# mauro3/KissMCMC.jl

Measured on AMD Instinct MI355X. Metric: walker-steps/sec, higher is better.
Workload: dtype f64

## Files before the change

include/kissmcmc_hip.h:

```cpp
#ifndef KISSMCMC_HIP_H
#define KISSMCMC_HIP_H

#include <stdint.h>

#ifdef __cplusplus
extern "C" {
#endif

#define KMC_VERSION 100

typedef enum kmc_status {
    KMC_OK = 0,
    KMC_ERR_A_SCALE = 1,
    KMC_ERR_ODD_WALKERS = 2,
    KMC_ERR_TOO_FEW_WALKERS = 3,
    KMC_ERR_BAD_ARG = 4,
    KMC_ERR_NONFINITE_LOGP = 5,
    KMC_ERR_HIP = 6,
    KMC_ERR_OOM = 7,
    KMC_ERR_NO_DEVICE = 8,
    KMC_ERR_UNSUPPORTED = 9
} kmc_status;

typedef enum kmc_density {
// ... 413 lines not shown
kmc_status  kmc_chain_psis_tail_reff(kmc_user_density* density, const double* params, const double* chain_host, int64_t nsamples, int64_t nwalkers,
                                     int64_t ndim, int64_t first_sample, const uint8_t* walker_mask, int64_t thin, const double* r_eff_j,
                                     int32_t split, int64_t max_lag, int64_t obs_first, int64_t obs_count, int64_t workspace_bytes, int device,
                                     double* tail, double* m_j, double* xc_j, int32_t* n_tail_j, int64_t* tail_len, double* r_eff_used,
                                     int64_t* tail_len_j, int64_t* n_reff_nan, int64_t* n_out);

kmc_status  kmc_debug_accept_terms(uint64_t seed, uint64_t step, uint64_t walker0, int64_t n, int64_t nhalf, double a_scale,
                                   int64_t ndim, int device, int64_t* partner_host, double* z_host, double* t1_host, double* lu_host);
kmc_status  kmc_debug_chain_by_walker(const void* src_host, int is_float, int64_t K, int64_t nl, int64_t ld, int64_t nd, int64_t w0,
                                      int64_t nw, int64_t dst_stride, double* dst_host, int64_t dst_len, int device);
kmc_status  kmc_debug_rows_compact(const double* src_host, int64_t rows, int64_t ld, int64_t nd, double* dst_host, int64_t dst_len,
                                   int device);
int         kmc_debug_phase_spec(int density, int L, int K, int iter);
int         kmc_debug_shared_draws(int density, int L, int K, int iter);
int         kmc_debug_replay_variant(int density, int64_t nwalkers, int64_t ndim, int64_t nburnin, int64_t g0, int64_t n, int moments, int chain);

#ifdef __cplusplus
}
#endif
#endif
```

kissmcmc.jl_amd/_lib.py:

```python
from __future__ import annotations

import ctypes as C
import os

_HERE = os.path.dirname(os.path.abspath(__file__))
LIB_PATH = os.environ.get("KMC_LIB_PATH") or os.path.join(_HERE, "libkissmcmc_hip.so")

OK, ERR_A_SCALE, ERR_ODD_WALKERS, ERR_TOO_FEW_WALKERS, ERR_BAD_ARG, ERR_NONFINITE_LOGP, \
    ERR_HIP, ERR_OOM, ERR_NO_DEVICE, ERR_UNSUPPORTED = range(10)
GAUSSIAN_ISO, EXPONENTIAL, ROSENBROCK, LOGNORMAL, MVNORMAL2 = range(5)
USER_DENSITY = 100
HOST_DENSITY = 101
DATA_DENSITY = 102
HOST_LOGPDF_FN = C.CFUNCTYPE(C.c_int, C.POINTER(C.c_double), C.c_int64, C.c_int64, C.POINTER(C.c_double), C.c_void_p)
HOST_PROPOSE_FN = C.CFUNCTYPE(C.c_int, C.POINTER(C.c_double), C.c_int64, C.c_int64, C.POINTER(C.c_double), C.c_void_p)
HOST_ACCEPTED_FN = C.CFUNCTYPE(C.c_int, C.POINTER(C.c_uint8), C.c_int64, C.c_int64, C.c_int64, C.c_int32, C.c_void_p)
F64 = 0
F32 = 1
STORE_CHAIN, STORE_LOGP, MOMENTS, NO_GRAPH, P2P, ISLANDS, P2P_FINEGRAINED, P2P_PUSH = 1, 2, 4, 8, 16, 64, 128, 512
STREAM_CHAIN = 2048
CHAIN_BY_WALKER = 4096
STORE_BLOBS = 8192
MOVE_STRETCH, MOVE_DE, MOVE_SNOOKER, MOVE_MIX = 0, 1, 3, 4
MIX_MAX = 4
# ... 5 lines not shown
RCCL_ID_BYTES = 128

SYMBOLS = [
    "kmc_version", "kmc_device_count", "kmc_last_error", "kmc_status_string", "kmc_validate",
    "kmc_g_pdf", "kmc_cdf_g_inv", "kmc_emcee_run", "kmc_sampler_create", "kmc_sampler_destroy",
    "kmc_sampler_set_stream", "kmc_sampler_bind_positions", "kmc_sampler_p2p_export", "kmc_sampler_p2p_connect", "kmc_sampler_p2p_connect_local", "kmc_sampler_p2p_link_probe", "kmc_sampler_set_positions", "kmc_sampler_init_ball", "kmc_sampler_set_state", "kmc_sampler_run", "kmc_sampler_half_step",
    "kmc_sampler_sync", "kmc_sampler_last_run_ms", "kmc_sampler_generation", "kmc_sampler_nsamples",
    "kmc_sampler_launch_count", "kmc_sampler_describe", "kmc_sampler_device_ptr", "kmc_sampler_get_positions",
    "kmc_sampler_get_logp", "kmc_sampler_get_naccept", "kmc_sampler_get_accept_ratio",
    "kmc_sampler_get_moments", "kmc_sampler_get_chain", "kmc_sampler_get_chain_by_walker", "kmc_logpdf_eval", "kmc_logpdf_eval_host",
    "kmc_user_density_create", "kmc_user_density_create_body", "kmc_user_density_destroy", "kmc_metropolis_validate", "kmc_metropolis_run", "kmc_cholesky_lower", "kmc_int_acorr", "kmc_sampler_int_acorr",
    "kmc_sizeof_config", "kmc_sizeof_metropolis_config", "kmc_sizeof_outputs", "kmc_sizeof_metropolis_outputs", "kmc_deal_seed", "kmc_deal_perm", "kmc_sampler_deal_pack", "kmc_sampler_deal_unpack",
    "kmc_sampler_get_walker_ids", "kmc_sampler_set_walker_ids", "kmc_sampler_set_chain_host", "kmc_rccl_unique_id", "kmc_sampler_rccl_init",
    "kmc_sampler_rccl_capture", "kmc_sampler_rccl_set_capture", "kmc_rccl_version", "kmc_device_free_bytes",
    "kmc_sampler_launch_mode", "kmc_updated_budget", "kmc_set_updated_budget_mb", "kmc_debug_accept_terms",
    "kmc_debug_chain_by_walker", "kmc_debug_rows_compact", "kmc_debug_phase_spec", "kmc_debug_shared_draws", "kmc_debug_replay_variant",
    "kmc_user_density_create_body_blob", "kmc_user_density_nblob", "kmc_logpdf_blob_eval_host", "kmc_sampler_get_blobs",
    "kmc_device_cache_release", "kmc_user_density_is_separable", "kmc_host_prefault", "kmc_data_density_create",
    "kmc_sampler_get_rung_state", "kmc_sampler_set_rung_state", "kmc_sampler_get_swaps",
    "kmc_sampler_get_rung_loglike", "kmc_sampler_set_rung_loglike_sum", "kmc_sampler_get_ladder", "kmc_sampler_set_ladder",
    "kmc_sampler_order_stats", "kmc_sampler_chain_argmax", "kmc_chain_order_stats", "kmc_chain_argmax",
    "kmc_sampler_histograms", "kmc_chain_histograms", "kmc_hist_pair_plan",
    "kmc_sampler_lag_sums", "kmc_chain_lag_sums", "kmc_convergence_stats", "kmc_sampler_convergence", "kmc_chain_convergence",
    "kmc_convergence_plan",
    "kmc_rank_plan", "kmc_rank_normal_scores", "kmc_sampler_rank_scores", "kmc_chain_rank_scores", "kmc_sampler_rank_convergence",
    "kmc_chain_rank_convergence",
    "kmc_sampler_hdi", "kmc_chain_hdi", "kmc_hdi_span",
    "kmc_sampler_covariance", "kmc_chain_covariance", "kmc_cov_plan", "kmc_cov_correlation",
    "kmc_sampler_pointwise_stats", "kmc_chain_pointwise_stats", "kmc_sampler_pointwise_loglike", "kmc_chain_pointwise_loglike",
    "kmc_pointwise_plan", "kmc_waic_stats",
    "kmc_sampler_psis_loo", "kmc_chain_psis_loo", "kmc_sampler_psis_tail", "kmc_chain_psis_tail", "kmc_psis_plan", "kmc_loo_stats",
# ... 285 lines not shown
    L.kmc_sampler_launch_mode.restype = C.c_int
    L.kmc_sampler_launch_mode.argtypes = [vp, C.POINTER(C.c_int)]
    L.kmc_updated_budget.restype = None
    L.kmc_updated_budget.argtypes = [ip, ip]
    L.kmc_set_updated_budget_mb.restype = None
    L.kmc_set_updated_budget_mb.argtypes = [C.c_double]
    L.kmc_debug_accept_terms.argtypes = [C.c_uint64, C.c_uint64, C.c_uint64, C.c_int64, C.c_int64, C.c_double, C.c_int64, C.c_int, ip, dp, dp, dp]
    L.kmc_debug_chain_by_walker.argtypes = [vp, C.c_int, C.c_int64, C.c_int64, C.c_int64, C.c_int64, C.c_int64, C.c_int64, C.c_int64, dp, C.c_int64, C.c_int]
    L.kmc_debug_rows_compact.argtypes = [dp, C.c_int64, C.c_int64, C.c_int64, dp, C.c_int64, C.c_int]
    L.kmc_debug_phase_spec.restype = C.c_int
    L.kmc_debug_phase_spec.argtypes = [C.c_int, C.c_int, C.c_int, C.c_int]
    L.kmc_debug_shared_draws.restype = C.c_int
    L.kmc_debug_shared_draws.argtypes = [C.c_int, C.c_int, C.c_int, C.c_int]
    L.kmc_debug_replay_variant.restype = C.c_int
    L.kmc_debug_replay_variant.argtypes = [C.c_int, C.c_int64, C.c_int64, C.c_int64, C.c_int64, C.c_int64, C.c_int, C.c_int]
    for fn, T in ((L.kmc_sizeof_config, Config), (L.kmc_sizeof_metropolis_config, MetropolisConfig),
                  (L.kmc_sizeof_outputs, Outputs), (L.kmc_sizeof_metropolis_outputs, MetropolisOutputs)):
        if fn() != C.sizeof(T):
            raise ImportError(f"{LIB_PATH}: struct layout mismatch ({fn.__name__}() = {fn()}, the ctypes mirror {T.__name__} is {C.sizeof(T)} bytes): "
                              "rebuild the library or update kissmcmc_jl_amd/_lib.py from include/kissmcmc_hip.h")
    _lib = L
    return L


def check(status: int) -> None:
    if status != OK:
        L = lib()
        msg = L.kmc_last_error().decode() or L.kmc_status_string(status).decode()
        raise KmcError(status, msg)
```

kissmcmc.jl_amd/build.py:

```python
from __future__ import annotations

import os
import shutil
import subprocess

_HERE = os.path.dirname(os.path.abspath(__file__))
CSRC = os.path.join(_HERE, "csrc")
LIB = os.path.join(_HERE, "libkissmcmc_hip.so")
SOURCES = ["kmc_sampler.hip", "kmc_validate.hip", "kmc_describe.hip", "kmc_plan.hip", "kmc_launch.hip", "kmc_updated.hip", "kmc_state.hip", "kmc_copy.hip", "kmc_rtc.hip", "kmc_p2p.hip", "kmc_metropolis_api.hip", "kmc_acorr.hip", "kmc_summary.hip", "kmc_hist.hip", "kmc_convergence.hip", "kmc_rank.hip", "kmc_hdi.hip", "kmc_cov.hip", "kmc_pointwise.hip", "kmc_rccl.hip", "kmc_diag.hip", "kmc_inst_host.hip", "kmc_inst_host_temper.hip", "kmc_inst_host_temper_snooker.hip", "kmc_data.hip"] + \
          [f"kmc_inst_{d}{part}.hip" for part in ("", "_var", "_p2p", "_lds", "_spec", "_share", "_de", "_snooker", "_temper", "_temper_snooker") for d in ("lognormal", "exponential", "gaussian_iso", "rosenbrock", "mvnormal2")
           if (part, d) != ("_share", "mvnormal2")]
HEADERS = ["kmc_psis_fit.hpp", "kmc_host.hpp", "kmc_sampler.hpp", "kmc_device.hpp", "kmc_kernels.hpp", "kmc_islands.hpp", "kmc_generation.hpp", "kmc_copy_kernels.hpp", "kmc_summary_kernels.hpp", "kmc_hist_kernels.hpp", "kmc_convergence_kernels.hpp", "kmc_convergence_host.hpp", "kmc_rank_kernels.hpp", "kmc_rank_host.hpp", "kmc_hdi_kernels.hpp", "kmc_cov_kernels.hpp", "kmc_chain_view.hpp", "kmc_chain_kernels.hpp", "kmc_metropolis.hpp", "kmc_tables.hpp", "kmc_shared_draws.hpp", "kmc_recognise.hpp", "kmc_data.hpp", "kmc_pointwise.hpp", os.path.join("..", "..", "include", "kissmcmc_hip.h")]
PRELOAD = ["-mllvm", "-amdgpu-kernarg-preload-count=14"]
FLAGS = ["--offload-arch=gfx950", "-O3", "-std=c++17", "-fPIC", "-ffp-contract=off",
         "-fvisibility=hidden", "-Wall", "-Wno-unused-function"]


def _hipcc() -> str:
    for c in (shutil.which("hipcc"), "/opt/rocm/bin/hipcc"):
        if c and os.path.exists(c):
            return c
    raise RuntimeError("hipcc not found: the HIP library cannot be built")




def stale(lib: str = LIB) -> bool:
# ... 38 lines not shown
```

kissmcmc.jl_amd/csrc/kmc_describe.hip:

```cpp
#include <cstdio>
#include <sstream>

#include "kmc_sampler.hpp"

using namespace kmc;
using namespace kmc_host;

namespace {
std::string launch_mode_text(const kmc_sampler* s, const char* what)
{
    std::string t = ((s->cfg.flags & KMC_NO_GRAPH) || s->launch_mode == 2) ? std::string(", eager launches (") + what + " among the preloaded kernel parameters)"
                    : s->launch_mode == 3 ? ", hipGraph replay of " + std::to_string(s->uchunk) + " generations with per-replay parameter updates (" + what + " preloaded)"
                                          : std::string(", hipGraph replay of 64 generations");
    if (s->calib_graph_ms > 0.f) {
        char b[128];
        std::snprintf(b, sizeof(b), " (measured per 64 generations: table graph %.3f ms, %s %.3f ms)", s->calib_graph_ms, s->launch_mode == 2 ? "eager launches" : "updated graph", s->calib_eager_ms);
        t += b;
    }
    return t;
}

void write_islands(std::ostringstream& o, const kmc_sampler* s)
{
    o << "island mode: " << s->nislands << " islands of " << s->island_size << " walkers in LDS, " << s->island_gens
// ... 51 lines not shown
}
void write_route(std::ostringstream& o, const kmc_sampler* s)
{
    if (s->islands) write_islands(o, s);
    else if (s->resident) write_resident(o, s);
    else if (s->fused) write_generation(o, s);
    else if (s->data_eval) write_data_density(o, s);
    else if (s->host_eval) write_host_density(o, s);
    else if (s->plan.vec) write_two_launch_vec(o, s);
    else write_two_launch_generic(o, s);
}

void write_feed_stats(std::ostringstream& o, const kmc_sampler* s)
{
    if (s->feed_replays <= 0 || !debug_opt("feed-stats")) return;
    char b[200];
    std::snprintf(b, sizeof(b), "; feeding thread per replay of %lld generations: wait for a free executable %.1f us, parameter updates %.1f us, hipGraphLaunch %.1f us (%lld replays)",
                  (long long)s->uchunk, s->feed_wait_ns / 1e3 / s->feed_replays, s->feed_update_ns / 1e3 / s->feed_replays, s->feed_launch_ns / 1e3 / s->feed_replays, (long long)s->feed_replays);
    o << b;
}

std::string move_kernel(const kmc_sampler* s, const char* stem)
{
    const std::string k = std::string("half_step_") + stem;
    return s->host_eval ? k + "_generic (propose / accept passes)" : s->plan.vec ? k + "_vec" : k + "_generic";
}
void write_move(std::ostringstream& o, const kmc_sampler* s)
{
    char b[160];
    if (s->cfg.move == KMC_MOVE_DE) {
        std::snprintf(b, sizeof(b), "; differential-evolution move (KMC_MOVE_DE): gamma0 %.6g, sigma %.3g, kernel ", de_gamma0_of(s->cfg), s->cfg.de_sigma);
        o << b << move_kernel(s, "de");
    }
    if (s->cfg.move == KMC_MOVE_SNOOKER) {
// ... 85 lines not shown
}
}

KMC_EXPORT kmc_status kmc_sampler_describe(const kmc_sampler* s, char* buf, int64_t buflen)
{
    if (!s || !buf || buflen <= 0) return fail(KMC_ERR_BAD_ARG, "bad argument");
    std::ostringstream o;
    write_route(o, s);
    write_feed_stats(o, s);
    write_move(o, s);
    write_tempering(o, s);
    write_storage(o, s);
    write_density(o, s);
    write_shard(o, s);
    write_geometry(o, s);
    const std::string t = o.str();
    std::snprintf(buf, (size_t)buflen, "%s", t.c_str());
    return KMC_OK;
}
```

kissmcmc.jl_amd/csrc/kmc_launch.hip:

```cpp
#include <algorithm>
#include <cmath>
#include <cstdio>
#include <cstdlib>

#define KMC_DEFINE_LAUNCH_KERNELS
#include "kmc_sampler.hpp"

using namespace kmc;
using namespace kmc_host;

namespace kmc_host {

template <int L, int K, int ITER, class T>
FlushFn flush_one()
{
    if constexpr (ITER <= L && ITER * K <= 16) return flush_moments_vec<L, K, ITER, T>;
    else return nullptr;
}

template <int L, int K>
FlushFn flush_iter(int iter, bool f32)
{
    switch (iter) {
    case 1: return f32 ? flush_one<L, K, 1, float>() : flush_one<L, K, 1, double>();
// ... 561 lines not shown
{
    if (s->fused) HIP_TRY(generation_settle(s));
    KMC_TRY(ensure_graph(s));
    if (!s->graph_exec) return eager_generations(s, kGraphChunk, left);
    KMC_TRY(sync_device_counter(s));
    KMC_TRY(chain_before(s, s->generation + kGraphChunk));
    HIP_TRY(hipGraphLaunch(s->graph_exec, s->stream));
    if (!s->fused) HIP_TRY(launch_sweep(s));
    s->generation += kGraphChunk;
    s->dev_gen += kGraphChunk;
    s->launches += (launches_per_generation(s) + (s->temper ? 1 : 0)) * kGraphChunk;
    *left -= kGraphChunk;
    return chain_after(s);
}

kmc_status updated_chunk(kmc_sampler* s, int64_t* left)
{
    if (s->fused) HIP_TRY(generation_settle(s));
    KMC_TRY(chain_before(s, s->generation + s->uchunk));
    bool launched = false;
    if (launch_updated_graph(s, &launched) != KMC_OK) {
        s->launch_mode = 1;
        if (debug_opt("feed-stats")) std::fprintf(stderr, "[kissmcmc_hip] the updated-graph replay failed (%s): table graph from here on\n", kmc_last_error());
        if (!launched) return KMC_OK;
        HIP_TRY(hipStreamSynchronize(s->stream));
    }
    if (!s->fused) HIP_TRY(launch_sweep(s));
    s->generation += s->uchunk;
    s->launches += launches_per_generation(s) * s->uchunk;
    *left -= s->uchunk;
    return chain_after(s);
}

inline int64_t calib_gens(const kmc_sampler* s) { return std::max<int64_t>(4 * kGraphChunk, 2 * s->uchunk); }
inline int64_t calib_min(const kmc_sampler* s) { return kGraphChunk + 2 * std::max<int64_t>(kGraphChunk, s->uchunk) + 2 * calib_gens(s) + kGraphChunk; }

kmc_status calibrate(kmc_sampler* s, bool with_updated, int64_t* left)
{
    hipEvent_t e0 = nullptr, e1 = nullptr, e2 = nullptr;
    HIP_TRY(hipEventCreate(&e0));
    HIP_TRY(hipEventCreate(&e1));
    HIP_TRY(hipEventCreate(&e2));
    const int64_t gens = calib_gens(s);
    kmc_status st = graph_chunk(s, left);
    if (st == KMC_OK) st = with_updated ? updated_chunk(s, left) : eager_generations(s, kGraphChunk, left);
    if (st == KMC_OK) st = with_updated ? updated_chunk(s, left) : eager_generations(s, kGraphChunk, left);
    if (st == KMC_OK && hipEventRecord(e0, s->stream) != hipSuccess) st = KMC_ERR_HIP;
    for (int64_t r = 0; r < gens / kGraphChunk && st == KMC_OK; ++r) st = graph_chunk(s, left);
    if (st == KMC_OK && hipEventRecord(e1, s->stream) != hipSuccess) st = KMC_ERR_HIP;
    if (with_updated) { for (int64_t r = 0; r < gens / s->uchunk && st == KMC_OK && s->launch_mode == 0; ++r) st = updated_chunk(s, left); }
    else if (st == KMC_OK) st = eager_generations(s, gens, left);
    if (st == KMC_OK && hipEventRecord(e2, s->stream) != hipSuccess) st = KMC_ERR_HIP;
    float tg = 0.f, tu = 0.f;
    if (st == KMC_OK && (hipEventSynchronize(e2) != hipSuccess || hipEventElapsedTime(&tg, e0, e1) != hipSuccess ||
                         hipEventElapsedTime(&tu, e1, e2) != hipSuccess)) st = KMC_ERR_HIP;
    (void)hipEventDestroy(e0); (void)hipEventDestroy(e1); (void)hipEventDestroy(e2);
    if (st != KMC_OK) return st == KMC_ERR_HIP ? fail(st, "launch-mode calibration failed") : st;
    if (s->launch_mode == 0) {
        s->launch_mode = tu < 0.98f * tg ? (with_updated ? 3 : 2) : 1;
        s->calib_graph_ms = tg * (float)kGraphChunk / (float)gens; s->calib_eager_ms = tu * (float)kGraphChunk / (float)gens;
    }
    return KMC_OK;
}

enum class LaunchEnv { none, graph, eager, updated, updated_budget };
LaunchEnv launch_env()
{
    static const char* const names[] = {"graph", "eager", "updated", "updated,budget"};
    const char* const e = std::getenv("KMC_LAUNCH");
    for (int i = 0; e && i < 4; ++i)
        if (std::strcmp(e, names[i]) == 0) return (LaunchEnv)(i + 1);
    return LaunchEnv::none;
}

kmc_status decide_launch_mode(kmc_sampler* s, LaunchEnv env, bool use_graph, int64_t* left)
{
    constexpr int64_t kWorthMeasuring = 4096;
    const bool long_job = s->cfg.ngenerations >= kWorthMeasuring || s->generation + *left >= kWorthMeasuring;
    const bool updated_asked = env == LaunchEnv::updated || env == LaunchEnv::updated_budget;
    if (use_graph && s->launch_mode == 0 && s->user && updated_graph_possible(s) && !s->uexec[0][0] && (updated_asked || (long_job && *left >= calib_min(s)))) {
        if (ensure_updated_graph(s) != KMC_OK) {
            (void)hipGetLastError();
            drop_updated_graph(s);
            s->updated_refused = true;
        }
    }
    if (s->temper && updated_asked) s->temper_updated_fallback = true;
    if (!use_graph || s->launch_mode != 0) return KMC_OK;
    if (env == LaunchEnv::graph) s->launch_mode = 1;
    else if (env == LaunchEnv::eager) s->launch_mode = 2;
    else if (env == LaunchEnv::updated && updated_graph_possible(s)) { s->launch_mode = 3; s->updated_forced = true; }
    else if (env == LaunchEnv::updated_budget && updated_graph_possible(s) && update_budget_left(s)) s->launch_mode = 3;
    else if (!updated_graph_possible(s)) s->launch_mode = 1;
    else if (*left >= calib_min(s) && long_job) {
        const bool room = update_budget_left(s);
        if (!room) note_budget_spent(s);
        KMC_TRY(calibrate(s, room, left));
    }
    return KMC_OK;
}

kmc_status run_launches(kmc_sampler* s, int64_t ngen)
{
    if (s->fused && s->fused_L > 0 && ngen > 0 && !(s->pos2_current && s->own_pos && !s->pos_exposed)) {
        HIP_TRY(generation_settle(s));
        HIP_TRY(hipMemcpyAsync(s->d_pos2, s->d_pos, (size_t)s->nrows * (size_t)s->ld * sizeof(double), hipMemcpyDeviceToDevice, s->stream));
        HIP_TRY(hipMemcpyAsync(s->d_logp2, s->d_logp, (size_t)s->nrows * sizeof(double), hipMemcpyDeviceToDevice, s->stream));
        s->pos2_current = true;
    }
    int64_t left = ngen;
    bool use_graph = !(s->cfg.flags & KMC_NO_GRAPH);
    if (s->comm && !s->comm_graph_ok) use_graph = false;
    KMC_TRY(decide_launch_mode(s, launch_env(), use_graph, &left));
    while (use_graph && s->launch_mode == 3 && left >= s->uchunk) {
        if (!s->updated_forced && !update_budget_left(s)) {
            note_budget_spent(s);
            s->launch_mode = 0;
            if (left >= calib_min(s)) KMC_TRY(calibrate(s, false, &left));
            break;
        }
        KMC_TRY(updated_chunk(s, &left));
    }
    if (s->launch_mode == 2) use_graph = false;
    while (use_graph && left >= kGraphChunk) KMC_TRY(graph_chunk(s, &left));
    KMC_TRY(eager_generations(s, left, &left));
    if (s->fused) HIP_TRY(generation_settle(s));
    return KMC_OK;
}

}

KMC_EXPORT kmc_status kmc_sampler_run(kmc_sampler* s, int64_t ngen)
{
    if (!s || ngen < 0) return fail(KMC_ERR_BAD_ARG, "bad argument");
    if (!s->positions_set) return fail(KMC_ERR_BAD_ARG, "kmc_sampler_set_positions has not succeeded yet");
    if (s->cfg.shard_count != 1 && !s->p2p && !s->comm)
        return fail(KMC_ERR_UNSUPPORTED, "kmc_sampler_run needs shard_count == 1, KMC_P2P or an RCCL communicator (kmc_sampler_rccl_init); "
                                         "other replica-sharded drivers call kmc_sampler_half_step and exchange themselves");
    if (s->p2p && !s->connected) return fail(KMC_ERR_BAD_ARG, "kmc_sampler_p2p_connect has not been called");
    if (s->generation + ngen >= (int64_t)1 << 31) return fail(KMC_ERR_UNSUPPORTED, "at most 2^31 - 1 generations (the step index is 32 bits)");
// ... 65 lines not shown
```

kissmcmc.jl_amd/csrc/kmc_sampler.hpp:

```cpp
#pragma once
#include <string>
#include <utility>
#include <vector>

#include "kmc_host.hpp"

KMC_EXPORT int kmc_version(void);

namespace kmc_host {

static_assert(1024 % kmc::kDrawBatch == 0, "the draw table holds whole batches");
constexpr int64_t kDrawTableGens = 1024;
constexpr int64_t kGraphChunk = 64;
constexpr int kUExec = 6;
enum : int { kVarGeneric = 0, kVarCredit = 1, kVarShareBurnin = 2, kUVariants = 3 };
constexpr size_t kGuardBytes = 4096;
constexpr int kHostPieces = 8;
constexpr size_t kResidentLdsMax = 156 * 1024;

struct Plan {
    kmc::HalfStepFn fn = nullptr;
    kmc::HalfStepFn fn_credit = nullptr;
    kmc::HalfStepFn fn_share_burnin = nullptr;
    int share_burnin = 0;
    bool vec = false;
    bool ragged = false;
    int L = 1, K = 1, ITER = 1;
};

struct UserKernels {
// ... 97 lines not shown
    bool dst_chain_reg = false, dst_logp_reg = false;
    int64_t blocks_copied = 0;
    int64_t blocks_waited = 0;
    void* comm = nullptr;
    bool comm_graph_ok = true;
    uint32_t* d_ids = nullptr;
    uint64_t user_seed = 0;
    int64_t moment_base = 0;
    int64_t generation = 0;
    int64_t dev_gen = 0;
    int64_t launches = 0;
    int launch_mode = 0;
    float calib_graph_ms = 0.f, calib_eager_ms = 0.f;
    hipGraphExec_t graph_exec = nullptr;
    hipGraph_t graph = nullptr;
    hipGraph_t ugraph[kmc_host::kUVariants] = {};
    hipGraphExec_t uexec[kmc_host::kUVariants][kmc_host::kUExec] = {};
    hipEvent_t udone[kmc_host::kUExec] = {};
    bool uinflight[kmc_host::kUExec] = {};
    int unext = 0;
    std::vector<hipGraphNode_t> unodes[kmc_host::kUVariants];
    int64_t uchunk = 128;
    bool updated_forced = false;
    int64_t feed_wait_ns = 0, feed_update_ns = 0, feed_launch_ns = 0, feed_replays = 0;
    unsigned vec_lds = 0;
    bool updated_refused = false;
    bool budget_fallback = false;
    std::vector<kmc_host::DevAlloc> allocs;
    hipEvent_t ev0 = nullptr, ev1 = nullptr;
    bool have_run_events = false;
    bool positions_set = false;
    bool host_eval = false;
    double* d_prop = nullptr;
    double* d_p1 = nullptr;
    double* h_prop = nullptr;
    double* h_p1 = nullptr;
    double* h_prop_dev = nullptr;
    double* h_p1_dev = nullptr;
    uint8_t* d_acc = nullptr;
// ... 87 lines not shown

kmc_status ensure_graph(kmc_sampler* s);
kmc_status flush_moments_now(kmc_sampler* s);
kmc_status unfuse(kmc_sampler* s);
kmc::DrawConsts draw_consts(const kmc_sampler* s);
kmc::HalfStepArgs make_args(const kmc_sampler* s, int half, bool graph_mode, int64_t gen_offset);
kmc::HalfStepFront front_of(const kmc::HalfStepArgs& a, bool ragged_vec);
kmc::GenerationArgs make_generation_args(const kmc_sampler* s, int from, bool graph_mode, int64_t gen_offset);
kmc::GenerationFront generation_front_of(const kmc::GenerationArgs& a, int tpb);

bool updated_graph_possible(const kmc_sampler* s);
bool spec_variant_possible(const kmc_sampler* s, int variant, const char** why_not = nullptr);
int variant_share(const kmc_sampler* s, int variant);
int spec_of_chunk(const kmc_sampler* s, int64_t g0, int64_t n);
kmc_status ensure_updated_graph(kmc_sampler* s);
kmc_status launch_updated_graph(kmc_sampler* s, bool* launched);
void drop_updated_graph(kmc_sampler* s);
bool update_budget_left(const kmc_sampler* s);
void note_budget_spent(kmc_sampler* s);

hipError_t upload_rows(const kmc_sampler* s, double* dst_dev, const double* src_host, size_t rows);
hipError_t download_rows(const kmc_sampler* s, double* dst_host, const double* src_dev, size_t rows);
kmc_status chain_before(kmc_sampler* s, int64_t g_end);
kmc_status chain_after(kmc_sampler* s);
kmc_status chain_flush(kmc_sampler* s);
void chain_unregister(kmc_sampler* s);

kmc_status load_user(kmc_user_density* ud, const UserModuleSpec& spec, UserKernels* uk);
void set_offline_compiler_hint(bool wanted);
bool body_vec_possible(const kmc_user_density* ud, int64_t ndim);

kmc_status load_data(kmc_user_density* ud, int64_t ndim, DataKernels* dk);
std::string data_functor_source(const kmc_user_density* ud);
// ... 12 lines not shown
```

kissmcmc.jl_amd/csrc/kmc_updated.hip:

```cpp
#include <atomic>
#include <chrono>
#include <cstdio>

#include "kmc_sampler.hpp"

using namespace kmc;
using namespace kmc_host;

namespace kmc_host {

namespace {
struct ParamPack {
    HalfStepFront hf;
    HalfStepArgs ha;
    GenerationFront gf;
    GenerationArgs ga;
    void* ptrs[11];
    explicit ParamPack(bool fused)
    {
        if (fused) {
            ptrs[0] = &gf.sched; ptrs[1] = &gf.pin; ptrs[2] = &gf.lin; ptrs[3] = &gf.pout; ptrs[4] = &gf.seed_lo; ptrs[5] = &gf.seed_hi;
            ptrs[6] = &gf.h; ptrs[7] = &gf.nb; ptrs[8] = &gf.ld; ptrs[9] = &gf.gen; ptrs[10] = &ga;
        } else {
            ptrs[0] = &hf.pos; ptrs[1] = &hf.sched; ptrs[2] = &hf.ring_now; ptrs[3] = &hf.logp; ptrs[4] = &hf.gw0; ptrs[5] = &hf.nact_half;
// ... 32 lines not shown
        np.func = s->user ? reinterpret_cast<void*>(s->uk.vec) : reinterpret_cast<void*>(variant_fn(s, variant));
        np.gridDim = dim3((unsigned)s->grid);
        np.blockDim = dim3((unsigned)s->tpb);
        if (const int share = variant_share(s, variant); share > 0) {
            np.gridDim = dim3((unsigned)(s->h_loc / variant_walkers_per_wg(s, variant)));
            np.blockDim = dim3(64u * (unsigned)share);
        }
        np.sharedMemBytes = s->user ? s->vec_lds : 0u;
    }
    np.kernelParams = pk->ptrs;
    np.extra = nullptr;
    return np;
}

template <class Visit>
kmc_status for_each_node(const kmc_sampler* s, int variant, int64_t g0, Visit&& visit)
{
    ParamPack pk(s->fused);
    const int64_t per_gen = launches_per_generation(s);
    for (int64_t k = 0; k < per_gen * s->uchunk; ++k) {
        const int64_t g = k / per_gen;
        if (s->fused) {
            pk.ga = make_generation_args(s, (int)(g & 1), false, g0 + g);
            pk.gf = generation_front_of(pk.ga, s->fused_tpb);
        } else {
            pk.ha = make_args(s, (int)(k & 1), false, g0 + g);
            pk.hf = front_of(pk.ha, s->ragged_vec());
        }
        KMC_TRY(visit(k, node_params(s, variant, &pk)));
    }
    return KMC_OK;
}
}

void drop_updated_graph(kmc_sampler* s)
{
    for (int i = 0; i < kUExec; ++i) {
        for (int v = 0; v < kUVariants; ++v)
            if (s->uexec[v][i]) { (void)hipGraphExecDestroy(s->uexec[v][i]); s->uexec[v][i] = nullptr; }
        if (s->udone[i]) { (void)hipEventDestroy(s->udone[i]); s->udone[i] = nullptr; }
        s->uinflight[i] = false;
    }
    s->unext = 0;
    for (int v = 0; v < kUVariants; ++v)
        if (s->ugraph[v]) { (void)hipGraphDestroy(s->ugraph[v]); s->ugraph[v] = nullptr; }
}

bool spec_variant_possible(const kmc_sampler* s, int variant, const char** why_not)
{
    const char* why = nullptr;
    std::string v;
    const bool credits = variant == kVarCredit;
    if (variant == kVarGeneric) return true;
    if (debug_opt("spec", &v) && v == "0") why = "KMC_DEBUG=spec=0";
    else if (variant == kVarShareBurnin && debug_opt("share", &v) && v == "0") why = "KMC_DEBUG=share=0";
    else if (s->user || s->fused || s->host_eval || !s->plan.vec) why = "not the two-launch vector route of a menu density";
    else if (variant_fn(s, variant) == nullptr) why = "no instance for this move, row type or geometry";
    else if (s->h_loc != (int64_t)s->grid * variant_walkers_per_wg(s, kVarGeneric) || s->h_loc % variant_walkers_per_wg(s, variant) != 0) why = "grid not full";
    else if (credits && !s->d_msum) why = "moments off";
    else if (credits && (s->d_chain || s->d_chain_logp || s->d_chain_blob)) why = "chain on";
// ... 4 lines not shown
int spec_of_chunk(const kmc_sampler* s, int64_t g0, int64_t n)
{
    if (g0 >= s->cfg.nburnin) return spec_variant_possible(s, kVarCredit) ? kVarCredit : kVarGeneric;
    if (g0 + n <= s->cfg.nburnin && spec_variant_possible(s, kVarShareBurnin)) return kVarShareBurnin;
    return kVarGeneric;
}

bool updated_graph_possible(const kmc_sampler* s)
{
    if (s->p2p || s->host_eval || s->islands || s->resident || s->comm || s->updated_refused) return false;
    if (s->temper) return false;
    if (s->fused) return s->user ? s->uk.generation != nullptr : s->generation_kernel != nullptr;
    return s->user ? (s->plan.vec && s->uk.vec != nullptr) : s->plan.fn != nullptr;
}

kmc_status ensure_updated_graph(kmc_sampler* s)
{
    if (s->uexec[kVarGeneric][0]) return KMC_OK;
    for (int v = 0; v < kUVariants; ++v) {
        if (!spec_variant_possible(s, v)) continue;
        HIP_TRY(hipGraphCreate(&s->ugraph[v], 0));
        s->unodes[v].assign((size_t)(launches_per_generation(s) * s->uchunk), nullptr);
        hipGraphNode_t prev = nullptr;
        KMC_TRY(for_each_node(s, v, 0, [&](int64_t k, const hipKernelNodeParams& np) -> kmc_status {
            hipGraphNode_t node = nullptr;
            HIP_TRY(hipGraphAddKernelNode(&node, s->ugraph[v], prev ? &prev : nullptr, prev ? 1 : 0, &np));
            s->unodes[v][(size_t)k] = node;
            prev = node;
            return KMC_OK;
        }));
        for (int i = 0; i < kUExec; ++i) HIP_TRY(hipGraphInstantiate(&s->uexec[v][i], s->ugraph[v], nullptr, nullptr, 0));
    }
    for (int i = 0; i < kUExec; ++i) HIP_TRY(hipEventCreateWithFlags(&s->udone[i], hipEventDisableTiming));
    return KMC_OK;
}

namespace {
double update_bytes_each()
{
    static const double b = [] {
        int v = 0;
        return (hipRuntimeGetVersion(&v) == hipSuccess && v >= 70200000) ? 2.0 : 80.0;
    }();
    return b;
}
std::atomic<int64_t> g_update_calls{0};
std::atomic<int64_t>& update_budget()
{
    static std::atomic<int64_t> budget{[] {
        double mb = 64.0;
        std::string v;
        if (debug_opt("updated-budget-mb", &v) && !v.empty()) mb = std::atof(v.c_str());
        return (int64_t)(mb * 1048576.0 / update_bytes_each());
    }()};
    return budget;
}
}

bool update_budget_left(const kmc_sampler* s)
{
    return g_update_calls.load(std::memory_order_relaxed) + launches_per_generation(s) * s->uchunk <= update_budget().load(std::memory_order_relaxed);
}

void note_budget_spent(kmc_sampler* s)
{
    s->budget_fallback = true;
    static std::atomic<bool> said{false};
    if (!said.exchange(true))
        std::fprintf(stderr, "[kissmcmc_hip] the updated-graph launch mode has used up this process's budget (%lld parameter updates, "
                             "kmc_set_updated_budget_mb / KMC_DEBUG=updated-budget-mb=n; this HIP runtime keeps ~%.0f B per update): samplers now "
                             "choose between the table graph and eager launches (up to ~9 %% slower per half-step; results are identical)\n",
                     (long long)g_update_calls.load(std::memory_order_relaxed), update_bytes_each());
}

kmc_status launch_updated_graph(kmc_sampler* s, bool* launched)
{
    *launched = false;
    KMC_TRY(ensure_updated_graph(s));
    g_update_calls.fetch_add(launches_per_generation(s) * s->uchunk, std::memory_order_relaxed);
    const int i = s->unext;
    int v = spec_of_chunk(s, s->generation, s->uchunk);
    if (!s->uexec[v][i]) v = kVarGeneric;
    const auto t_wait0 = std::chrono::steady_clock::now();
    if (s->uinflight[i]) { HIP_TRY(hipEventSynchronize(s->udone[i])); s->uinflight[i] = false; }
    const auto t_upd0 = std::chrono::steady_clock::now();
    KMC_TRY(for_each_node(s, v, s->generation, [&](int64_t k, const hipKernelNodeParams& np) -> kmc_status {
        HIP_TRY(hipGraphExecKernelNodeSetParams(s->uexec[v][i], s->unodes[v][(size_t)k], &np));
        return KMC_OK;
    }));
    const auto t_upd1 = std::chrono::steady_clock::now();
    HIP_TRY(hipGraphLaunch(s->uexec[v][i], s->stream));
    const auto t_launch1 = std::chrono::steady_clock::now();
    s->feed_wait_ns += std::chrono::duration_cast<std::chrono::nanoseconds>(t_upd0 - t_wait0).count();
    s->feed_update_ns += std::chrono::duration_cast<std::chrono::nanoseconds>(t_upd1 - t_upd0).count();
    s->feed_launch_ns += std::chrono::duration_cast<std::chrono::nanoseconds>(t_launch1 - t_upd1).count();
    s->feed_replays += 1;
    *launched = true;
    HIP_TRY(hipEventRecord(s->udone[i], s->stream));
    s->uinflight[i] = true;
    s->unext = (i + 1) % kUExec;
    return KMC_OK;
}

}

KMC_EXPORT void kmc_updated_budget(int64_t* calls_used, int64_t* calls_budget)
{
    if (calls_used) *calls_used = g_update_calls.load(std::memory_order_relaxed);
    if (calls_budget) *calls_budget = update_budget().load(std::memory_order_relaxed);
}

KMC_EXPORT void kmc_set_updated_budget_mb(double mb)
{
    update_budget().store(mb <= 0.0 ? 0 : (int64_t)(mb * 1048576.0 / update_bytes_each()), std::memory_order_relaxed);
}
```

Baseline: 9.076 billion.

## Add long updated-graph replays of 256 generations alongside the short ring

Adds a second ring of updated-graph executables covering 256 generations, used whenever the remaining work and the burn-in boundary allow it, and otherwise falls back to the 128-generation ring. Longer replays are meant to amortise per-replay host costs such as hipGraphLaunch, event waits and executable turnover across more generations. In exchange it costs extra graph instantiation time and memory, and the long graph is only built when at least two long replays are ahead. A small planner header and a debug export are added to expose the replay schedule.

Result: no change. 9.138 billion (median of 6 runs) (+0.7%).

```diff
diff --git a/include/kissmcmc_hip.h b/include/kissmcmc_hip.h
--- a/include/kissmcmc_hip.h
+++ b/include/kissmcmc_hip.h
@@ -451,6 +451,7 @@
 int         kmc_debug_phase_spec(int density, int L, int K, int iter);
 int         kmc_debug_shared_draws(int density, int L, int K, int iter);
 int         kmc_debug_replay_variant(int density, int64_t nwalkers, int64_t ndim, int64_t nburnin, int64_t g0, int64_t n, int moments, int chain);
+int64_t     kmc_debug_replay_plan(int64_t generation, int64_t left, int64_t nburnin, int64_t short_len, int64_t long_len, int long_ready);
 
 #ifdef __cplusplus
 }
diff --git a/kissmcmc.jl_amd/_lib.py b/kissmcmc.jl_amd/_lib.py
--- a/kissmcmc.jl_amd/_lib.py
+++ b/kissmcmc.jl_amd/_lib.py
@@ -43,7 +43,7 @@
     "kmc_sampler_get_walker_ids", "kmc_sampler_set_walker_ids", "kmc_sampler_set_chain_host", "kmc_rccl_unique_id", "kmc_sampler_rccl_init",
     "kmc_sampler_rccl_capture", "kmc_sampler_rccl_set_capture", "kmc_rccl_version", "kmc_device_free_bytes",
     "kmc_sampler_launch_mode", "kmc_updated_budget", "kmc_set_updated_budget_mb", "kmc_debug_accept_terms",
-    "kmc_debug_chain_by_walker", "kmc_debug_rows_compact", "kmc_debug_phase_spec", "kmc_debug_shared_draws", "kmc_debug_replay_variant",
+    "kmc_debug_chain_by_walker", "kmc_debug_rows_compact", "kmc_debug_phase_spec", "kmc_debug_shared_draws", "kmc_debug_replay_variant", "kmc_debug_replay_plan",
     "kmc_user_density_create_body_blob", "kmc_user_density_nblob", "kmc_logpdf_blob_eval_host", "kmc_sampler_get_blobs",
     "kmc_device_cache_release", "kmc_user_density_is_separable", "kmc_host_prefault", "kmc_data_density_create",
     "kmc_sampler_get_rung_state", "kmc_sampler_set_rung_state", "kmc_sampler_get_swaps",
@@ -359,6 +359,8 @@
     L.kmc_debug_shared_draws.argtypes = [C.c_int, C.c_int, C.c_int, C.c_int]
     L.kmc_debug_replay_variant.restype = C.c_int
     L.kmc_debug_replay_variant.argtypes = [C.c_int, C.c_int64, C.c_int64, C.c_int64, C.c_int64, C.c_int64, C.c_int, C.c_int]
+    L.kmc_debug_replay_plan.restype = C.c_int64
+    L.kmc_debug_replay_plan.argtypes = [C.c_int64, C.c_int64, C.c_int64, C.c_int64, C.c_int64, C.c_int]
     for fn, T in ((L.kmc_sizeof_config, Config), (L.kmc_sizeof_metropolis_config, MetropolisConfig),
                   (L.kmc_sizeof_outputs, Outputs), (L.kmc_sizeof_metropolis_outputs, MetropolisOutputs)):
         if fn() != C.sizeof(T):
diff --git a/kissmcmc.jl_amd/build.py b/kissmcmc.jl_amd/build.py
--- a/kissmcmc.jl_amd/build.py
+++ b/kissmcmc.jl_amd/build.py
@@ -10,7 +10,7 @@
 SOURCES = ["kmc_sampler.hip", "kmc_validate.hip", "kmc_describe.hip", "kmc_plan.hip", "kmc_launch.hip", "kmc_updated.hip", "kmc_state.hip", "kmc_copy.hip", "kmc_rtc.hip", "kmc_p2p.hip", "kmc_metropolis_api.hip", "kmc_acorr.hip", "kmc_summary.hip", "kmc_hist.hip", "kmc_convergence.hip", "kmc_rank.hip", "kmc_hdi.hip", "kmc_cov.hip", "kmc_pointwise.hip", "kmc_rccl.hip", "kmc_diag.hip", "kmc_inst_host.hip", "kmc_inst_host_temper.hip", "kmc_inst_host_temper_snooker.hip", "kmc_data.hip"] + \
           [f"kmc_inst_{d}{part}.hip" for part in ("", "_var", "_p2p", "_lds", "_spec", "_share", "_de", "_snooker", "_temper", "_temper_snooker") for d in ("lognormal", "exponential", "gaussian_iso", "rosenbrock", "mvnormal2")
            if (part, d) != ("_share", "mvnormal2")]
-HEADERS = ["kmc_psis_fit.hpp", "kmc_host.hpp", "kmc_sampler.hpp", "kmc_device.hpp", "kmc_kernels.hpp", "kmc_islands.hpp", "kmc_generation.hpp", "kmc_copy_kernels.hpp", "kmc_summary_kernels.hpp", "kmc_hist_kernels.hpp", "kmc_convergence_kernels.hpp", "kmc_convergence_host.hpp", "kmc_rank_kernels.hpp", "kmc_rank_host.hpp", "kmc_hdi_kernels.hpp", "kmc_cov_kernels.hpp", "kmc_chain_view.hpp", "kmc_chain_kernels.hpp", "kmc_metropolis.hpp", "kmc_tables.hpp", "kmc_shared_draws.hpp", "kmc_recognise.hpp", "kmc_data.hpp", "kmc_pointwise.hpp", os.path.join("..", "..", "include", "kissmcmc_hip.h")]
+HEADERS = ["kmc_psis_fit.hpp", "kmc_host.hpp", "kmc_sampler.hpp", "kmc_replay_plan.hpp", "kmc_device.hpp", "kmc_kernels.hpp", "kmc_islands.hpp", "kmc_generation.hpp", "kmc_copy_kernels.hpp", "kmc_summary_kernels.hpp", "kmc_hist_kernels.hpp", "kmc_convergence_kernels.hpp", "kmc_convergence_host.hpp", "kmc_rank_kernels.hpp", "kmc_rank_host.hpp", "kmc_hdi_kernels.hpp", "kmc_cov_kernels.hpp", "kmc_chain_view.hpp", "kmc_chain_kernels.hpp", "kmc_metropolis.hpp", "kmc_tables.hpp", "kmc_shared_draws.hpp", "kmc_recognise.hpp", "kmc_data.hpp", "kmc_pointwise.hpp", os.path.join("..", "..", "include", "kissmcmc_hip.h")]
 PRELOAD = ["-mllvm", "-amdgpu-kernarg-preload-count=14"]
 FLAGS = ["--offload-arch=gfx950", "-O3", "-std=c++17", "-fPIC", "-ffp-contract=off",
          "-fvisibility=hidden", "-Wall", "-Wno-unused-function"]
diff --git a/kissmcmc.jl_amd/csrc/kmc_describe.hip b/kissmcmc.jl_amd/csrc/kmc_describe.hip
--- a/kissmcmc.jl_amd/csrc/kmc_describe.hip
+++ b/kissmcmc.jl_amd/csrc/kmc_describe.hip
@@ -89,10 +89,18 @@
 void write_feed_stats(std::ostringstream& o, const kmc_sampler* s)
 {
     if (s->feed_replays <= 0 || !debug_opt("feed-stats")) return;
-    char b[200];
-    std::snprintf(b, sizeof(b), "; feeding thread per replay of %lld generations: wait for a free executable %.1f us, parameter updates %.1f us, hipGraphLaunch %.1f us (%lld replays)",
-                  (long long)s->uchunk, s->feed_wait_ns / 1e3 / s->feed_replays, s->feed_update_ns / 1e3 / s->feed_replays, s->feed_launch_ns / 1e3 / s->feed_replays, (long long)s->feed_replays);
+    char b[240];
+    std::snprintf(b, sizeof(b), "; feeding thread per replay of %lld generations%s: wait for a free executable %.1f us, parameter updates %.1f us, hipGraphLaunch %.1f us (%lld replays)",
+                  (long long)(s->long_replays > 0 ? s->feed_gens / s->feed_replays : s->uchunk), s->long_replays > 0 ? " on average" : "",
+                  s->feed_wait_ns / 1e3 / s->feed_replays, s->feed_update_ns / 1e3 / s->feed_replays, s->feed_launch_ns / 1e3 / s->feed_replays, (long long)s->feed_replays);
     o << b;
+}
+
+void write_long_replays(std::ostringstream& o, const kmc_sampler* s)
+{
+    if (s->long_replays <= 0) return;
+    o << "; long replays of " << s->lring.gens << " generations where a call holds them, cut at nburnin (" << s->long_replays << " so far, "
+      << kUExecLong << " executables per kernel variant)";
 }
 
 std::string move_kernel(const kmc_sampler* s, const char* stem)
@@ -208,6 +216,7 @@
     write_density(o, s);
     write_shard(o, s);
     write_geometry(o, s);
+    write_long_replays(o, s);
     const std::string t = o.str();
     std::snprintf(buf, (size_t)buflen, "%s", t.c_str());
     return KMC_OK;
diff --git a/kissmcmc.jl_amd/csrc/kmc_launch.hip b/kissmcmc.jl_amd/csrc/kmc_launch.hip
--- a/kissmcmc.jl_amd/csrc/kmc_launch.hip
+++ b/kissmcmc.jl_amd/csrc/kmc_launch.hip
@@ -4,6 +4,7 @@
 #include <cstdlib>
 
 #define KMC_DEFINE_LAUNCH_KERNELS
+#include "kmc_replay_plan.hpp"
 #include "kmc_sampler.hpp"
 
 using namespace kmc;
@@ -599,21 +600,21 @@
     return chain_after(s);
 }
 
-kmc_status updated_chunk(kmc_sampler* s, int64_t* left)
+kmc_status updated_chunk(kmc_sampler* s, int64_t gens, int64_t* left)
 {
     if (s->fused) HIP_TRY(generation_settle(s));
-    KMC_TRY(chain_before(s, s->generation + s->uchunk));
+    KMC_TRY(chain_before(s, s->generation + gens));
     bool launched = false;
-    if (launch_updated_graph(s, &launched) != KMC_OK) {
+    if (launch_updated_graph(s, gens, &launched) != KMC_OK) {
         s->launch_mode = 1;
         if (debug_opt("feed-stats")) std::fprintf(stderr, "[kissmcmc_hip] the updated-graph replay failed (%s): table graph from here on\n", kmc_last_error());
         if (!launched) return KMC_OK;
         HIP_TRY(hipStreamSynchronize(s->stream));
     }
     if (!s->fused) HIP_TRY(launch_sweep(s));
-    s->generation += s->uchunk;
-    s->launches += launches_per_generation(s) * s->uchunk;
-    *left -= s->uchunk;
+    s->generation += gens;
+    s->launches += launches_per_generation(s) * gens;
+    *left -= gens;
     return chain_after(s);
 }
 
@@ -628,12 +629,12 @@
     HIP_TRY(hipEventCreate(&e2));
     const int64_t gens = calib_gens(s);
     kmc_status st = graph_chunk(s, left);
-    if (st == KMC_OK) st = with_updated ? updated_chunk(s, left) : eager_generations(s, kGraphChunk, left);
-    if (st == KMC_OK) st = with_updated ? updated_chunk(s, left) : eager_generations(s, kGraphChunk, left);
+    if (st == KMC_OK) st = with_updated ? updated_chunk(s, s->uchunk, left) : eager_generations(s, kGraphChunk, left);
+    if (st == KMC_OK) st = with_updated ? updated_chunk(s, s->uchunk, left) : eager_generations(s, kGraphChunk, left);
     if (st == KMC_OK && hipEventRecord(e0, s->stream) != hipSuccess) st = KMC_ERR_HIP;
     for (int64_t r = 0; r < gens / kGraphChunk && st == KMC_OK; ++r) st = graph_chunk(s, left);
     if (st == KMC_OK && hipEventRecord(e1, s->stream) != hipSuccess) st = KMC_ERR_HIP;
-    if (with_updated) { for (int64_t r = 0; r < gens / s->uchunk && st == KMC_OK && s->launch_mode == 0; ++r) st = updated_chunk(s, left); }
+    if (with_updated) { for (int64_t r = 0; r < gens / s->uchunk && st == KMC_OK && s->launch_mode == 0; ++r) st = updated_chunk(s, s->uchunk, left); }
     else if (st == KMC_OK) st = eager_generations(s, gens, left);
     if (st == KMC_OK && hipEventRecord(e2, s->stream) != hipSuccess) st = KMC_ERR_HIP;
     float tg = 0.f, tu = 0.f;
@@ -663,7 +664,7 @@
     constexpr int64_t kWorthMeasuring = 4096;
     const bool long_job = s->cfg.ngenerations >= kWorthMeasuring || s->generation + *left >= kWorthMeasuring;
     const bool updated_asked = env == LaunchEnv::updated || env == LaunchEnv::updated_budget;
-    if (use_graph && s->launch_mode == 0 && s->user && updated_graph_possible(s) && !s->uexec[0][0] && (updated_asked || (long_job && *left >= calib_min(s)))) {
+    if (use_graph && s->launch_mode == 0 && s->user && updated_graph_possible(s) && !s->uring.built() && (updated_asked || (long_job && *left >= calib_min(s)))) {
         if (ensure_updated_graph(s) != KMC_OK) {
             (void)hipGetLastError();
             drop_updated_graph(s);
@@ -675,10 +676,10 @@
     if (env == LaunchEnv::graph) s->launch_mode = 1;
     else if (env == LaunchEnv::eager) s->launch_mode = 2;
     else if (env == LaunchEnv::updated && updated_graph_possible(s)) { s->launch_mode = 3; s->updated_forced = true; }
-    else if (env == LaunchEnv::updated_budget && updated_graph_possible(s) && update_budget_left(s)) s->launch_mode = 3;
+    else if (env == LaunchEnv::updated_budget && updated_graph_possible(s) && update_budget_left(s, s->uchunk)) s->launch_mode = 3;
     else if (!updated_graph_possible(s)) s->launch_mode = 1;
     else if (*left >= calib_min(s) && long_job) {
-        const bool room = update_budget_left(s);
+        const bool room = update_budget_left(s, s->uchunk);
         if (!room) note_budget_spent(s);
         KMC_TRY(calibrate(s, room, left));
     }
@@ -697,18 +698,26 @@
     bool use_graph = !(s->cfg.flags & KMC_NO_GRAPH);
     if (s->comm && !s->comm_graph_ok) use_graph = false;
     KMC_TRY(decide_launch_mode(s, launch_env(), use_graph, &left));
-    while (use_graph && s->launch_mode == 3 && left >= s->uchunk) {
-        if (!s->updated_forced && !update_budget_left(s)) {
+    int64_t long_len = long_replay_length(s);
+    while (use_graph && s->launch_mode == 3) {
+        if (long_len > 0 && !s->updated_forced && !update_budget_left(s, long_len)) long_len = 0;
+        const int64_t gens = replay_plan_next(s->generation, left, s->cfg.nburnin, s->uchunk, long_len, s->lring.built());
+        if (gens == kReplayRemainder) break;
+        if (gens != s->uchunk && !ensure_long_graph(s, gens)) { long_len = 0; continue; }
+        if (!s->updated_forced && !update_budget_left(s, gens)) {
             note_budget_spent(s);
             s->launch_mode = 0;
             if (left >= calib_min(s)) KMC_TRY(calibrate(s, false, &left));
             break;
         }
-        KMC_TRY(updated_chunk(s, &left));
+        KMC_TRY(updated_chunk(s, gens, &left));
     }
     if (s->launch_mode == 2) use_graph = false;
     while (use_graph && left >= kGraphChunk) KMC_TRY(graph_chunk(s, &left));
     KMC_TRY(eager_generations(s, left, &left));
+    if (use_graph && s->launch_mode == 3 && long_len > 0 && !s->lring.built() &&
+        replay_plan_long_ahead(s->generation, s->cfg.ngenerations - s->generation, s->cfg.nburnin, s->uchunk, long_len, kReplayLongWorth) >= kReplayLongWorth)
+        (void)ensure_long_graph(s, long_len);
     if (s->fused) HIP_TRY(generation_settle(s));
     return KMC_OK;
 }
diff --git a/kissmcmc.jl_amd/csrc/kmc_replay_plan.hpp b/kissmcmc.jl_amd/csrc/kmc_replay_plan.hpp
--- /dev/null
+++ b/kissmcmc.jl_amd/csrc/kmc_replay_plan.hpp
@@ -0,0 +1,40 @@
+#pragma once
+#include <cstdint>
+
+namespace kmc_host {
+
+constexpr int64_t kReplayRemainder = 0;
+constexpr int kReplayLongWorth = 2;
+
+inline bool replay_fits_one_side(int64_t g, int64_t left, int64_t nburnin, int64_t len)
+{
+    return len > 0 && left >= len && (g >= nburnin || len <= nburnin - g);
+}
+
+inline int64_t replay_plan_step(int64_t g, int64_t left, int64_t nburnin, int64_t short_len, int64_t long_len)
+{
+    if (replay_fits_one_side(g, left, nburnin, long_len)) return long_len;
+    if (short_len > 0 && left >= short_len) return short_len;
+    return kReplayRemainder;
+}
+
+inline int replay_plan_long_ahead(int64_t g, int64_t left, int64_t nburnin, int64_t short_len, int64_t long_len, int enough)
+{
+    int n = 0;
+    while (n < enough) {
+        const int64_t len = replay_plan_step(g, left, nburnin, short_len, long_len);
+        if (len == kReplayRemainder) break;
+        if (len == long_len) ++n;
+        g += len;
+        left -= len;
+    }
+    return n;
+}
+
+inline int64_t replay_plan_next(int64_t g, int64_t left, int64_t nburnin, int64_t short_len, int64_t long_len, bool long_ready)
+{
+    if (long_len > 0 && !long_ready && replay_plan_long_ahead(g, left, nburnin, short_len, long_len, kReplayLongWorth) < kReplayLongWorth) long_len = 0;
+    return replay_plan_step(g, left, nburnin, short_len, long_len);
+}
+
+}
diff --git a/kissmcmc.jl_amd/csrc/kmc_sampler.hpp b/kissmcmc.jl_amd/csrc/kmc_sampler.hpp
--- a/kissmcmc.jl_amd/csrc/kmc_sampler.hpp
+++ b/kissmcmc.jl_amd/csrc/kmc_sampler.hpp
@@ -13,7 +13,20 @@
 constexpr int64_t kDrawTableGens = 1024;
 constexpr int64_t kGraphChunk = 64;
 constexpr int kUExec = 6;
+constexpr int kUExecLong = 3;
+constexpr int64_t kLongReplay = 256;
 enum : int { kVarGeneric = 0, kVarCredit = 1, kVarShareBurnin = 2, kUVariants = 3 };
+struct UpdatedRing {
+    int64_t gens = 0;
+    int nexec = 0;
+    hipGraph_t graph[kUVariants] = {};
+    hipGraphExec_t exec[kUVariants][kUExec] = {};
+    hipEvent_t done[kUExec] = {};
+    bool inflight[kUExec] = {};
+    int next = 0;
+    std::vector<hipGraphNode_t> nodes[kUVariants];
+    bool built() const { return exec[kVarGeneric][0] != nullptr; }
+};
 constexpr size_t kGuardBytes = 4096;
 constexpr int kHostPieces = 8;
 constexpr size_t kResidentLdsMax = 156 * 1024;
@@ -141,15 +154,14 @@
     float calib_graph_ms = 0.f, calib_eager_ms = 0.f;
     hipGraphExec_t graph_exec = nullptr;
     hipGraph_t graph = nullptr;
-    hipGraph_t ugraph[kmc_host::kUVariants] = {};
-    hipGraphExec_t uexec[kmc_host::kUVariants][kmc_host::kUExec] = {};
-    hipEvent_t udone[kmc_host::kUExec] = {};
-    bool uinflight[kmc_host::kUExec] = {};
-    int unext = 0;
-    std::vector<hipGraphNode_t> unodes[kmc_host::kUVariants];
+    kmc_host::UpdatedRing uring;
     int64_t uchunk = 128;
+    kmc_host::UpdatedRing lring;
+    bool long_refused = false;
+    int64_t long_replays = 0;
     bool updated_forced = false;
     int64_t feed_wait_ns = 0, feed_update_ns = 0, feed_launch_ns = 0, feed_replays = 0;
+    int64_t feed_gens = 0;
     unsigned vec_lds = 0;
     bool updated_refused = false;
     bool budget_fallback = false;
@@ -267,9 +279,11 @@
 int variant_share(const kmc_sampler* s, int variant);
 int spec_of_chunk(const kmc_sampler* s, int64_t g0, int64_t n);
 kmc_status ensure_updated_graph(kmc_sampler* s);
-kmc_status launch_updated_graph(kmc_sampler* s, bool* launched);
+kmc_status launch_updated_graph(kmc_sampler* s, int64_t gens, bool* launched);
 void drop_updated_graph(kmc_sampler* s);
-bool update_budget_left(const kmc_sampler* s);
+bool update_budget_left(const kmc_sampler* s, int64_t gens);
+int64_t long_replay_length(const kmc_sampler* s);
+bool ensure_long_graph(kmc_sampler* s, int64_t gens);
 void note_budget_spent(kmc_sampler* s);
 
 hipError_t upload_rows(const kmc_sampler* s, double* dst_dev, const double* src_host, size_t rows);
diff --git a/kissmcmc.jl_amd/csrc/kmc_updated.hip b/kissmcmc.jl_amd/csrc/kmc_updated.hip
--- a/kissmcmc.jl_amd/csrc/kmc_updated.hip
+++ b/kissmcmc.jl_amd/csrc/kmc_updated.hip
@@ -2,6 +2,7 @@
 #include <chrono>
 #include <cstdio>
 
+#include "kmc_replay_plan.hpp"
 #include "kmc_sampler.hpp"
 
 using namespace kmc;
@@ -70,11 +71,11 @@
 }
 
 template <class Visit>
-kmc_status for_each_node(const kmc_sampler* s, int variant, int64_t g0, Visit&& visit)
+kmc_status for_each_node(const kmc_sampler* s, int variant, int64_t gens, int64_t g0, Visit&& visit)
 {
     ParamPack pk(s->fused);
     const int64_t per_gen = launches_per_generation(s);
-    for (int64_t k = 0; k < per_gen * s->uchunk; ++k) {
+    for (int64_t k = 0; k < per_gen * gens; ++k) {
         const int64_t g = k / per_gen;
         if (s->fused) {
             pk.ga = make_generation_args(s, (int)(g & 1), false, g0 + g);
@@ -89,17 +90,26 @@
 }
 }
 
-void drop_updated_graph(kmc_sampler* s)
+namespace {
+void drop_ring(UpdatedRing* r)
 {
     for (int i = 0; i < kUExec; ++i) {
         for (int v = 0; v < kUVariants; ++v)
-            if (s->uexec[v][i]) { (void)hipGraphExecDestroy(s->uexec[v][i]); s->uexec[v][i] = nullptr; }
-        if (s->udone[i]) { (void)hipEventDestroy(s->udone[i]); s->udone[i] = nullptr; }
-        s->uinflight[i] = false;
-    }
-    s->unext = 0;
+            if (r->exec[v][i]) { (void)hipGraphExecDestroy(r->exec[v][i]); r->exec[v][i] = nullptr; }
+        if (r->done[i]) { (void)hipEventDestroy(r->done[i]); r->done[i] = nullptr; }
+        r->inflight[i] = false;
+    }
+    r->next = 0;
+    r->gens = 0;
     for (int v = 0; v < kUVariants; ++v)
-        if (s->ugraph[v]) { (void)hipGraphDestroy(s->ugraph[v]); s->ugraph[v] = nullptr; }
+        if (r->graph[v]) { (void)hipGraphDestroy(r->graph[v]); r->graph[v] = nullptr; }
+}
+}
+
+void drop_updated_graph(kmc_sampler* s)
+{
+    drop_ring(&s->uring);
+    drop_ring(&s->lring);
 }
 
 bool spec_variant_possible(const kmc_sampler* s, int variant, const char** why_not)
@@ -134,25 +144,46 @@
     return s->user ? (s->plan.vec && s->uk.vec != nullptr) : s->plan.fn != nullptr;
 }
 
-kmc_status ensure_updated_graph(kmc_sampler* s)
-{
-    if (s->uexec[kVarGeneric][0]) return KMC_OK;
+namespace {
+kmc_status ensure_ring(kmc_sampler* s, UpdatedRing* r, int64_t gens, int nexec)
+{
+    if (r->built()) return KMC_OK;
+    const auto t0 = std::chrono::steady_clock::now();
+    r->gens = gens;
+    r->nexec = nexec;
     for (int v = 0; v < kUVariants; ++v) {
         if (!spec_variant_possible(s, v)) continue;
-        HIP_TRY(hipGraphCreate(&s->ugraph[v], 0));
-        s->unodes[v].assign((size_t)(launches_per_generation(s) * s->uchunk), nullptr);
+        HIP_TRY(hipGraphCreate(&r->graph[v], 0));
+        r->nodes[v].assign((size_t)(launches_per_generation(s) * gens), nullptr);
         hipGraphNode_t prev = nullptr;
-        KMC_TRY(for_each_node(s, v, 0, [&](int64_t k, const hipKernelNodeParams& np) -> kmc_status {
+        KMC_TRY(for_each_node(s, v, gens, 0, [&](int64_t k, const hipKernelNodeParams& np) -> kmc_status {
             hipGraphNode_t node = nullptr;
-            HIP_TRY(hipGraphAddKernelNode(&node, s->ugraph[v], prev ? &prev : nullptr, prev ? 1 : 0, &np));
-            s->unodes[v][(size_t)k] = node;
+            HIP_TRY(hipGraphAddKernelNode(&node, r->graph[v], prev ? &prev : nullptr, prev ? 1 : 0, &np));
+            r->nodes[v][(size_t)k] = node;
             prev = node;
             return KMC_OK;
         }));
-        for (int i = 0; i < kUExec; ++i) HIP_TRY(hipGraphInstantiate(&s->uexec[v][i], s->ugraph[v], nullptr, nullptr, 0));
-    }
-    for (int i = 0; i < kUExec; ++i) HIP_TRY(hipEventCreateWithFlags(&s->udone[i], hipEventDisableTiming));
+        for (int i = 0; i < nexec; ++i) HIP_TRY(hipGraphInstantiate(&r->exec[v][i], r->graph[v], nullptr, nullptr, 0));
+    }
+    for (int i = 0; i < nexec; ++i) HIP_TRY(hipEventCreateWithFlags(&r->done[i], hipEventDisableTiming));
+    if (debug_opt("feed-stats"))
+        std::fprintf(stderr, "[kissmcmc_hip] updated graph of %lld generations: %d executables per kernel variant built in %.2f ms\n", (long long)gens, nexec,
+                     std::chrono::duration_cast<std::chrono::microseconds>(std::chrono::steady_clock::now() - t0).count() / 1e3);
     return KMC_OK;
+}
+}
+
+kmc_status ensure_updated_graph(kmc_sampler* s)
+{
+    return ensure_ring(s, &s->uring, s->uchunk, kUExec);
+}
+
+int64_t long_replay_length(const kmc_sampler* s)
+{
+    if (s->stream_chain || s->d_mring || s->long_refused) return 0;
+    const long n = debug_opt_long("long-replay", (long)kLongReplay);
+    if (n < 2 || n > (1 << 20) || (n & ~1L) == s->uchunk) return 0;
+    return s->lring.built() ? s->lring.gens : (int64_t)(n & ~1L);
 }
 
 namespace {
@@ -177,9 +208,9 @@
 }
 }
 
-bool update_budget_left(const kmc_sampler* s)
-{
-    return g_update_calls.load(std::memory_order_relaxed) + launches_per_generation(s) * s->uchunk <= update_budget().load(std::memory_order_relaxed);
+bool update_budget_left(const kmc_sampler* s, int64_t gens)
+{
+    return g_update_calls.load(std::memory_order_relaxed) + launches_per_generation(s) * gens <= update_budget().load(std::memory_order_relaxed);
 }
 
 void note_budget_spent(kmc_sampler* s)
@@ -193,32 +224,46 @@
                      (long long)g_update_calls.load(std::memory_order_relaxed), update_bytes_each());
 }
 
-kmc_status launch_updated_graph(kmc_sampler* s, bool* launched)
+bool ensure_long_graph(kmc_sampler* s, int64_t gens)
+{
+    if (ensure_ring(s, &s->lring, gens, kUExecLong) == KMC_OK) return true;
+    (void)hipGetLastError();
+    drop_ring(&s->lring);
+    s->long_refused = true;
+    return false;
+}
+
+kmc_status launch_updated_graph(kmc_sampler* s, int64_t gens, bool* launched)
 {
     *launched = false;
-    KMC_TRY(ensure_updated_graph(s));
-    g_update_calls.fetch_add(launches_per_generation(s) * s->uchunk, std::memory_order_relaxed);
-    const int i = s->unext;
-    int v = spec_of_chunk(s, s->generation, s->uchunk);
-    if (!s->uexec[v][i]) v = kVarGeneric;
+    const bool is_long = gens != s->uchunk;
+    UpdatedRing* const r = is_long ? &s->lring : &s->uring;
+    if (!is_long) KMC_TRY(ensure_updated_graph(s));
+    if (r->gens != gens || !r->built()) return fail(KMC_ERR_BAD_ARG, "launch_updated_graph: no graph of this length (ensure_long_graph builds the long one)");
+    g_update_calls.fetch_add(launches_per_generation(s) * gens, std::memory_order_relaxed);
+    const int i = r->next;
+    int v = spec_of_chunk(s, s->generation, gens);
+    if (!r->exec[v][i]) v = kVarGeneric;
     const auto t_wait0 = std::chrono::steady_clock::now();
-    if (s->uinflight[i]) { HIP_TRY(hipEventSynchronize(s->udone[i])); s->uinflight[i] = false; }
+    if (r->inflight[i]) { HIP_TRY(hipEventSynchronize(r->done[i])); r->inflight[i] = false; }
     const auto t_upd0 = std::chrono::steady_clock::now();
-    KMC_TRY(for_each_node(s, v, s->generation, [&](int64_t k, const hipKernelNodeParams& np) -> kmc_status {
-        HIP_TRY(hipGraphExecKernelNodeSetParams(s->uexec[v][i], s->unodes[v][(size_t)k], &np));
+    KMC_TRY(for_each_node(s, v, gens, s->generation, [&](int64_t k, const hipKernelNodeParams& np) -> kmc_status {
+        HIP_TRY(hipGraphExecKernelNodeSetParams(r->exec[v][i], r->nodes[v][(size_t)k], &np));
         return KMC_OK;
     }));
     const auto t_upd1 = std::chrono::steady_clock::now();
-    HIP_TRY(hipGraphLaunch(s->uexec[v][i], s->stream));
+    HIP_TRY(hipGraphLaunch(r->exec[v][i], s->stream));
     const auto t_launch1 = std::chrono::steady_clock::now();
     s->feed_wait_ns += std::chrono::duration_cast<std::chrono::nanoseconds>(t_upd0 - t_wait0).count();
     s->feed_update_ns += std::chrono::duration_cast<std::chrono::nanoseconds>(t_upd1 - t_upd0).count();
     s->feed_launch_ns += std::chrono::duration_cast<std::chrono::nanoseconds>(t_launch1 - t_upd1).count();
     s->feed_replays += 1;
+    s->feed_gens += gens;
+    if (is_long) s->long_replays += 1;
     *launched = true;
-    HIP_TRY(hipEventRecord(s->udone[i], s->stream));
-    s->uinflight[i] = true;
-    s->unext = (i + 1) % kUExec;
+    HIP_TRY(hipEventRecord(r->done[i], s->stream));
+    r->inflight[i] = true;
+    r->next = (i + 1) % r->nexec;
     return KMC_OK;
 }
 
@@ -234,3 +279,8 @@
 {
     update_budget().store(mb <= 0.0 ? 0 : (int64_t)(mb * 1048576.0 / update_bytes_each()), std::memory_order_relaxed);
 }
+
+KMC_EXPORT int64_t kmc_debug_replay_plan(int64_t generation, int64_t left, int64_t nburnin, int64_t short_len, int64_t long_len, int long_ready)
+{
+    return replay_plan_next(generation, left, nburnin, short_len, long_len, long_ready != 0);
+}
```
